# Martinsos/edlib

Measured on NVIDIA H100. Metric: GCUPS, higher is better.
Workload: dtype u32

## Files before the change

edlib_b200/csrc/eb_common.h:

```cpp
#pragma once
#include <stdint.h>

#if defined(__CUDACC__)
#define EB_HD __host__ __device__ __forceinline__
#define EB_D __device__ __forceinline__
#else
#define EB_HD inline
#define EB_D inline
#endif

namespace eb {

struct U2 { uint32_t x, y; };

constexpr int KPOS = 4;

struct Rec {
    int best;
    int cnt;
    int last;
    int rsv;
    int pos[KPOS];
};

// ... 211 lines not shown
    int maxLen;
    int Ls;
    int Lidx, sigma, numKeys;
    const int* bucketStart;
    const int* positions;
    int maxBucket;
    int level;
    int spread;
    int* winPair;
    int* winK;
    int* winStart;
    int* winLen;
    int* winTf;
    int winCap;
    int* winCount;
    SeedPlan* plan;
};
struct Leftover {
    int pair;
    int excl;
};
enum RecState : int { REC_DONE = 100, REC_PENDING = 101 };
struct WinReduceParams {
    const SeedPlan* plan;
    const WinRec* winRecs;
    int numReads;
    Rec* out;
    int* extra;
    int* extraCount;
    int extraCap;
    const Ovf* ovf;
    const int* ovfCount;
    int ovfCap;
    Leftover* leftover;
    int* leftoverCount;
    const int* readList;
    int firstPair;
    const int* qlen;
    int kBound;
};
struct FinParams {
    const Rec* recs;
    const int* extra;
    const int* readList;
    int firstPair;
    int numReads;
    const int* qlen;
    int kBound;
    int* ed;
    int* endCount;
    long long* endStart;
    int* cnt32;
    int* pool;
    long long poolBase;
    int poolCap;
    int* header;
    const int* winCount;
};

enum ResStage : int {
    RS_LOC_COUNT = 0,
    RS_LOC_JOBS = 1,
    RS_LOC_APPLY = 2,
    RS_PATH_FLAG = 3,
    RS_PATH_JOBS = 4,
    RS_PATH_LEN = 5,
// ... 68 lines not shown
```

edlib_b200/csrc/eb_core.h:

```cpp
#pragma once
#include "eb_common.h"

#if defined(__CUDA_ARCH__)
#define EB_UNROLL _Pragma("unroll")
#else
#define EB_UNROLL
#endif

namespace eb {


EB_HD uint32_t funnel_l1(uint32_t lo, uint32_t hi) {
#if defined(__CUDA_ARCH__)
    return __funnelshift_l(lo, hi, 1);
#else
    return (hi << 1) | (lo >> 31);
#endif
}

EB_HD int popcount32(uint32_t v) {
#if defined(__CUDA_ARCH__)
    return __popc(v);
#else
    return __builtin_popcount(v);
// ... 633 lines not shown
        if (bandSlack >= 0) {
            while (i < c && E[i] - first <= bandSlack) last = E[i++];
        } else {
            while (i < c && E[i] - last <= K1_RANGE_GAP && E[i] - first <= p.spread) last = E[i++];
        }
        int lo = first - t, hi = last + t;
        if (lo <= prevHi) lo = prevHi + 1;
        if (lo < 0) lo = 0;
        if (hi > p.n - 1) hi = p.n - 1;
        if (lo > hi) continue;
        prevHi = hi;
        int ws = lo - (m + t);
        if (ws < 0) ws = 0;
        ws &= ~15;
        f(nW, ws, lo, hi);
        ++nW;
    }
    return nW;
}
EB_HD void seed_window_store(const SeedPlanParams& p, int w, int pair, int t, int ws, int lo, int hi) {
    p.winPair[w] = pair;
    p.winK[w] = t + 1;
    p.winStart[w] = ws;
    p.winLen[w] = hi - ws + 1;
    p.winTf[w] = lo - ws;
}

struct CoopSerial {
    static constexpr int W = 1;
    static EB_HD int lane() { return 0; }
    static EB_HD int width() { return 1; }
    static EB_HD void sync() {}
    static EB_HD bool any(bool v) { return v; }
    static EB_HD int add_shared(int* p, int v) {
        const int old = *p;
        *p = old + v;
        return old;
    }
    static EB_HD int scan(int v, int& total) {
        total = v;
        return 0;
    }
    static EB_HD int reserve(int* counter, int n) { return n > 0 ? atomic_add_int(counter, n) : 0; }
};

EB_HD constexpr int seed_ctl_words(int W) { return 2 + 3 * W; }
constexpr int SEED_CTL = seed_ctl_words(32);

template <int CAP, int K, class C>
EB_HD void seed_try(const SeedPlanParams& p, const uint8_t* q, int m, int Lk, const int (&pos)[K], const int (&a)[K],
                    int* E, int* ctl) {
    bool same[K];
    EB_UNROLL
    for (int k = 0; k < K; ++k) {
        same[k] = pos[k] >= 0 && pos[k] + p.Ls <= p.n;
        if (same[k]) {
            uint32_t diff = 0;
            for (int x = Lk; x < p.Ls; ++x) diff |= (uint32_t)(p.tcodes[pos[k] + x] ^ q[a[k] + x]);
            same[k] = diff == 0;
        }
    }
    EB_UNROLL
    for (int k = 0; k < K; ++k) {
        if (!same[k]) continue;
        const int at = C::add_shared(&ctl[0], 1);
        if (at < CAP) E[at] = pos[k] + (m - a[k]) - 1;
// ... 99 lines not shown
                        }
                    }
                    C::sync();
                }
            }
        }
    }
    int myWs = 0, myLo = 0, myHi = 0;
    const int nW = seed_windows(p, E, c, m, t, [&](int w, int ws, int lo, int hi) {
        if (w == lane) {
            myWs = ws;
            myLo = lo;
            myHi = hi;
        }
    });
    const int base = C::reserve(p.winCount, nW);
    if (nW > 0) {
        if (base + nW <= p.winCap) {
            if (lane < nW) seed_window_store(p, base + lane, pair, t, myWs, myLo, myHi);
            if (nW > W)
                seed_windows(p, E, c, m, t, [&](int w, int ws, int lo, int hi) {
                    if (w >= W && w % W == lane) seed_window_store(p, base + w, pair, t, ws, lo, hi);
                });
            pl.first = base;
            pl.count = nW;
            pl.state = SEED_WINDOWS;
        } else {
            pl.state = SEED_SATURATED;
        }
    }
    if (live && lane == 0) p.plan[slot] = pl;
}

EB_HD void win_reduce_read(const WinReduceParams& p, int slot) {
    const SeedPlan pl = p.plan[slot];
    Rec out;
    out.best = 0x7fffffff;
    out.cnt = 0;
    out.last = 0;
    out.rsv = pl.state;
    for (int q = 0; q < KPOS; ++q) out.pos[q] = 0;
    if (pl.state == SEED_WINDOWS) {
        const int t = pl.thr;
        int b = 0x7fffffff;
        for (int w = 0; w < pl.count; ++w) {
            const WinRec& r = p.winRecs[pl.first + w];
            if (r.cnt > 0 && r.best < b) b = r.best;
        }
        if (b > t) {
            out.rsv = SEED_NONE;
        } else {
            int total = 0;
            bool longList = false, listed = false;
            for (int w = 0; w < pl.count; ++w) {
                const WinRec& r = p.winRecs[pl.first + w];
                if (r.cnt <= 0 || r.best != b) continue;
                if (r.cnt > KPOSW) listed = true;
                total += r.cnt;
            }
            int listLen = 0;
            if (listed) {
                listLen = p.ovfCap > 0 ? *p.ovfCount : 0x7fffffff;
                if (listLen > p.ovfCap) longList = true;
            }
            int base = 0;
            if (!longList && total > KPOS) {
                base = atomic_add_int(p.extraCount, total - KPOS);
                if (base + total - KPOS > p.extraCap) longList = true;
            }
            if (longList) {
                out.rsv = SEED_LONG_LIST;
            } else {
                int i = 0;
                for (int w = 0; w < pl.count; ++w) {
                    const WinRec& r = p.winRecs[pl.first + w];
                    if (r.cnt <= 0 || r.best != b) continue;
                    for (int q = 0; q < r.cnt && q < KPOSW; ++q, ++i) {
                        if (i < KPOS) out.pos[i] = r.pos[q];
                        else p.extra[base + i - KPOS] = r.pos[q];
                    }
                    if (r.cnt > KPOSW) {
                        int found = 0;
                        for (int e = 0; e < listLen; ++e) {
                            const Ovf o = p.ovf[e];
                            if (o.rec != pl.first + w || o.score != b) continue;
                            if (found < r.cnt - KPOSW) p.extra[base + i++ - KPOS] = o.pos;
                            ++found;
                        }
                        if (found != r.cnt - KPOSW) longList = true;
                    }
                }
                if (longList) {
                    out.rsv = SEED_LONG_LIST;
                } else {
                    out.best = b;
                    out.cnt = total;
                    out.last = base;
                }
            }
        }
    }
    if (p.leftover) {
        const int pair = p.readList ? p.readList[slot] : p.firstPair + slot;
        const int m = p.qlen[pair];
        const int bound = (p.kBound < 0 || p.kBound > m) ? m : p.kBound;
        int excl = -3;
        if (out.rsv == SEED_WINDOWS) {
            out.rsv = REC_DONE;
        } else if (out.rsv == SEED_NONE && pl.thr >= 0 && pl.thr == bound) {
            out.rsv = REC_DONE;
        } else {
            excl = out.rsv == SEED_LONG_LIST ? -2 : (out.rsv == SEED_NONE ? pl.thr : -1);
            out.rsv = REC_PENDING;
        }
        if (excl != -3) {
            const int at = atomic_add_int(p.leftoverCount, 1);
            p.leftover[at].pair = pair;
            p.leftover[at].excl = excl;
        }
    }
    p.out[slot] = out;
}

EB_HD int hw_accepted_count(int best, int cnt, int m, int kBound, bool* minusOne) {
    *minusOne = false;
    if (best < 0 || best == 0x7fffffff || cnt <= 0) return -1;
    if (kBound >= 0 && best > kBound) return -1;
    if (best > m) return -1;
    const int W64 = (m + 63) / 64 * 64 - m;
    *minusOne = (best == m && W64 > 0);
    return cnt + (*minusOne ? 1 : 0);
}
EB_HD void fin_count_item(const FinParams& p, int slot) {
    const Rec r = p.recs[slot];
// ... 744 lines not shown
```

edlib_b200/csrc/eb_engine.cpp:

```cpp
#include "eb_engine_internal.h"

#include <sched.h>

namespace eb {

static int env_int(const char* name, int dflt) {
    const char* s = getenv(name);
    return (s && *s) ? atoi(s) : dflt;
}

static std::vector<int> parse_cpulist(const char* path) {
    std::vector<int> cpus;
    FILE* f = fopen(path, "r");
    if (!f) return cpus;
    char buf[4096];
    if (fgets(buf, sizeof(buf), f)) {
        for (char* tok = strtok(buf, ",\n"); tok; tok = strtok(nullptr, ",\n")) {
            int a = 0, b = 0;
            const int got = sscanf(tok, "%d-%d", &a, &b);
            if (got == 1) b = a;
            if (got >= 1)
                for (int c = a; c <= b && c < 4096; ++c) cpus.push_back(c);
        }
    }
// ... 29 lines not shown
    snprintf(path, sizeof(path), "/sys/devices/system/node/node%d/cpulist", node);
    std::vector<int> cpus = parse_cpulist(path);
    if (!cpus.empty() && HostPool::worker_cpus().empty()) HostPool::worker_cpus() = cpus;
}

EngineTunables::EngineTunables() {
    k1MinGroup = env_int("EDLIB_B200_K1_MIN_GROUP", k1MinGroup);
    k1MinChunk = env_int("EDLIB_B200_K1_MIN_CHUNK", k1MinChunk);
    ovfCap = env_int("EDLIB_B200_OVF_CAP", ovfCap);
    filterK0 = env_int("EDLIB_B200_FILTER_K0", filterK0);
    filterK1 = env_int("EDLIB_B200_FILTER_K1", filterK1);
    packParallelBytes = (size_t)env_int("EDLIB_B200_PACK_PARALLEL_KB", (int)(packParallelBytes >> 10)) << 10;
    filterSeedK = env_int("EDLIB_B200_FILTER_SEED_K", filterSeedK);
    filterSeedBucket = env_int("EDLIB_B200_FILTER_SEED_BUCKET", filterSeedBucket);
    filterSeedSlack = env_int("EDLIB_B200_FILTER_SEED_SLACK", filterSeedSlack);
    filterMinLevelReads = env_int("EDLIB_B200_FILTER_MIN_LEVEL_READS", filterMinLevelReads);
    tinySweepReads = env_int("EDLIB_B200_TINY_SWEEP_READS", tinySweepReads);
    filterSeedLevels = std::min(SEED_LEVELS, env_int("EDLIB_B200_FILTER_SEED_LEVELS", filterSeedLevels));
    filterMaxWindows = env_int("EDLIB_B200_FILTER_MAX_WINDOWS", filterMaxWindows);
    filterMinLen = env_int("EDLIB_B200_FILTER_MIN_LEN", filterMinLen);
    filterSpread = env_int("EDLIB_B200_FILTER_SPREAD", filterSpread);
    filterMinTarget = env_int("EDLIB_B200_FILTER_MIN_TARGET", filterMinTarget);
    filterSkipRepeats = env_int("EDLIB_B200_FILTER_SKIP_REPEATS", filterSkipRepeats);
    bandKernel = env_int("EDLIB_B200_BAND_KERNEL", bandKernel);
    collapseEqualities = env_int("EDLIB_B200_COLLAPSE_EQUALITIES", collapseEqualities);
    directUpload = env_int("EDLIB_B200_DIRECT_UPLOAD", directUpload);
    streamSlices = std::max(1, env_int("EDLIB_B200_STREAM_SLICES", streamSlices));
    directMinBytes = (size_t)env_int("EDLIB_B200_DIRECT_MIN_KB", (int)(directMinBytes >> 10)) << 10;
    deviceStage = env_int("EDLIB_B200_DEVICE_STAGE", deviceStage);
    windowCheckAfter = env_int("EDLIB_B200_WINDOW_CHECK", windowCheckAfter);
    longHwMinTarget = env_int("EDLIB_B200_LONG_HW_MIN_TARGET", longHwMinTarget);
    longSeedMaxK = env_int("EDLIB_B200_LONG_SEED_MAX_K", longSeedMaxK);
    devSliceReads = std::max(64, env_int("EDLIB_B200_SLICE_READS", devSliceReads));
    streamMinPairs = env_int("EDLIB_B200_STREAM_MIN_PAIRS", streamMinPairs);
    const int sliceMb = env_int("EDLIB_B200_SLICE_MB", 0);
    if (sliceMb > 0) sliceBytes = (size_t)sliceMb << 20;
    if (sliceMb > 0) pathSliceBytes = (size_t)sliceMb << 20;
    deviceResults = env_int("EDLIB_B200_DEVICE_RESULTS", deviceResults);
}

static int code_map(const uint32_t (&present)[8], uint8_t (&map)[256], int other) {
    int ncodes = 0;
    for (int b = 0; b < 256; ++b) ncodes += (present[b >> 5] >> (b & 31)) & 1u;
    int next = 0;
    for (int b = 0; b < 256; ++b) {
        if (present[b >> 5] >> (b & 31) & 1u) map[b] = (uint8_t)next++;
        else map[b] = (uint8_t)(other < 0 ? 0 : std::min(other, 255));
    }
    return ncodes;
}

Prepared* Engine::prepare(const BatchInput& in) {
    Backend* be = be_;
    Trace trace;
    Prepared* p = spare_ ? spare_ : new Prepared();
    spare_ = nullptr;
    try {
        p->bind(be);
        p->tg.clear();
        p->hasEq = false;
        p->ncodes = 0;
        p->computed = false;
        p->classified = false;
        p->ed.clear();
        p->endStart.clear();
        p->endCount.clear();
// ... 1110 lines not shown
```

edlib_b200/csrc/eb_engine.h:

```cpp
#pragma once
#include <stddef.h>
#include <stdint.h>

#include <map>
#include <string>
#include <utility>
#include <vector>

#include "../../include/edlib.h"
#include "eb_common.h"

namespace eb {

struct Backend {
    virtual ~Backend() {}
    virtual void* alloc(size_t bytes) = 0;
    virtual void free(void* p) = 0;
    virtual void* alloc_host(size_t bytes) = 0;
    virtual void free_host(void* p) = 0;
    virtual bool host_pinned(const void* , size_t ) { return false; }
    virtual void h2d(void* dst, const void* src, size_t bytes) = 0;
    virtual void d2h(void* dst, const void* src, size_t bytes) = 0;
    virtual void zero(void* dst, size_t bytes) = 0;
    virtual void d2d(void* dst, const void* src, size_t bytes) = 0;
// ... 28 lines not shown
    virtual void launch_seed_count(const SeedIndexParams& p) = 0;
    virtual void launch_scan(int* data, int count) = 0;
    virtual void launch_seed_fill(const SeedIndexParams& p) = 0;
    virtual void launch_seed_plan(const SeedPlanParams& p) = 0;
    virtual void launch_win_reduce(const WinReduceParams& p) = 0;
    virtual void launch_fin_count(const FinParams& p) = 0;
    virtual void launch_fin_fill(const FinParams& p) = 0;
    virtual void launch_qalpha(const QAlphaParams& p) = 0;
    virtual void reset_timing() = 0;
    virtual double kernel_ms(const char* nameOrNull) = 0;
    virtual int launches() = 0;
    virtual std::string kernel_report() = 0;
};

struct BatchInput {
    const char* const* queries;
    const int* queryLengths;
    const char* const* targets;
    const int* targetLengths;
    int numPairs;
    EdlibAlignConfig config;
};

struct EngineTunables {
    int k1MinGroup = 32;
    int k1MinChunk = 1024;
    int ovfCap = 1 << 20;
    size_t sliceBytes = 1ull << 30;
    size_t pathSliceBytes = 8ull << 30;
    int deviceResults = 1;
    size_t packParallelBytes = 32u << 20;
    int deviceStage = 1;
    int devSliceReads = 1 << 20;
    int streamSlices = 8;
    int streamMinPairs = 32768;
    int longHwMinTarget = 65536;
    int longSeedMaxK = 1024;
    int windowCheckAfter = 48;
    int filterSeedK = 20;
    int filterSeedBucket = 128;
    int filterSeedLevels = 4;
    int tinySweepReads = 8;
    int filterMinLevelReads = 64;
    int filterSeedSlack = 4;
    int filterK1 = 8;
    int filterK0 = 16;
    int filterMinLen = 96;
    int filterSpread = 1024;
    int filterMaxWindows = 32;
    int filterMinTarget = 65536;
    size_t directMinBytes = 1u << 20;
    int directUpload = 1;
    int collapseEqualities = 1;
    int bandKernel = 1;
    int filterSkipRepeats = 1;
    EngineTunables();
};

struct EngineStats {
    double kernelMs = 0;
    double k1Ms = 0;
    int launches = 0;
    long long h2dBytes = 0, d2hBytes = 0;
    long long k1Cells = 0;
    long long wCells = 0;
    long long filterDecided = 0, filterFallback = 0;
// ... 47 lines not shown
```

edlib_b200/csrc/eb_engine_internal.h:

```cpp
#pragma once
#include "eb_engine.h"

#include <stdio.h>
#include <stdlib.h>
#include <string.h>

#include <algorithm>
#include <cmath>
#include <exception>
#include <functional>
#include <atomic>
#include <condition_variable>
#include <mutex>
#include <chrono>
#include <map>
#include <stdexcept>
#include <thread>
#include <unordered_map>

namespace eb {


struct Trace {
    bool on;
// ... 382 lines not shown
    int firstPair = -1;
    size_t listOff = 0;
    int count = 0;
    long long poolBase = 0;
    int poolCap = 0;
    int poolFetched = 0;
    uint64_t done = 0;
    bool finished = false;
};

struct Pass {
    Engine& eng;
    Backend* be;
    Prepared* p;
    EngineTunables& tun;
    EngineStats& stats;
    Trace trace;
    const int N, mode, k;
    std::vector<int>&best, &cnt;
    std::vector<long long>& posStart;
    std::vector<int>&posLen, &posPool;
    std::vector<int> wPairs;
    std::vector<uint8_t> opsPool;
    WRunner runner;
    int laneOkCache[9] = {-1, -1, -1, -1, -1, -1, -1, -1, -1};

    bool devMode = false;
    std::vector<int> hostPairs;
    std::vector<DevSlice> slices;
    DevBuf<int> dEd, dEndCount, dHeaders, dPool, dLeftCount, dLists;
    DevBuf<long long> dEndStart;
    DevBuf<Leftover> dLeft;
    PinnedVec<int> hHeaders;
    long long poolReserved = 0;
    size_t listsUsed = 0;
    bool wholeArrays = false;
    long long windowsSeen = 0, readsSeen = 0;
    void* extraCopyDst = nullptr;
    const void* extraCopySrc = nullptr;
    size_t extraCopyBytes = 0;

    Pass(Engine& e, Backend* b, Prepared* pr)
        : eng(e), be(b), p(pr), tun(e.tun), stats(e.stats), N(pr->N), mode(pr->mode), k(pr->cfg.k),
          best(e.scratch.best), cnt(e.scratch.cnt), posStart(e.scratch.posStart), posLen(e.scratch.posLen),
          posPool(e.scratch.posPool), runner{&e, b, pr, &opsPool} {
        hHeaders.bind(b);
        best.resize((size_t)N);
        cnt.resize((size_t)N);
        posStart.resize((size_t)N);
        posLen.resize((size_t)N);
        posPool.clear();
    }
    void host_touch(const int* list, size_t n) {
        parallel_ranges(n, 65536, [&](size_t lo, size_t hi) {
            for (size_t i = lo; i < hi; ++i) {
                const int pair = list[i];
                best[pair] = -1;
                cnt[pair] = 0;
                posStart[pair] = -1;
                posLen[pair] = 0;
            }
        });
    }
    void host_touch_all() {
        parallel_ranges((size_t)N, 65536, [&](size_t lo, size_t hi) {
            for (size_t i = lo; i < hi; ++i) {
                best[i] = -1;
                cnt[i] = 0;
                posStart[i] = -1;
                posLen[i] = 0;
            }
        });
    }

    bool lane_ok(int m);

    void lane_launch(const std::vector<LJob>& jobs, int nw, int laneMode, bool rev, std::vector<Rec>& recs);

    template <class Sink>
// ... 126 lines not shown
```

edlib_b200/csrc/eb_kernels.cu:

```cuda
#include <cuda_runtime.h>
#include <ctype.h>
#include <stdio.h>
#include <sys/syscall.h>
#include <unistd.h>
#include <stdlib.h>
#include <string.h>

#include <algorithm>
#include <mutex>
#include <stdexcept>
#include <string>
#include <vector>

#include "eb_core.h"
#include "eb_engine.h"

namespace eb {

#if defined(__CUDA_ARCH__)
#define EB_DEV(expr, fallback) expr
#else
#define EB_DEV(expr, fallback) fallback
#endif
struct DevWarp {
// ... 322 lines not shown
}

__global__ void traceback_kernel(const TbParams p) {
    const int job = blockIdx.x * blockDim.x + threadIdx.x;
    if (job < p.numJobs) traceback_job(p, job);
}

__global__ void res_kernel(const ResParams p) {
    const int i = blockIdx.x * blockDim.x + threadIdx.x;
    if (i < p.numItems) res_item(p, i);
}

__global__ void split_kernel(const SplitParams p) {
    const int node = blockIdx.x * blockDim.x + threadIdx.x;
    if (node < p.numNodes) split_node(p, node);
}

__global__ void seed_count_kernel(const SeedIndexParams p) {
    const int i = blockIdx.x * blockDim.x + threadIdx.x;
    if (i < p.numPos) seed_count_item(p, i);
}
__global__ void seed_fill_kernel(const SeedIndexParams p) {
    const int i = blockIdx.x * blockDim.x + threadIdx.x;
    if (i < p.numPos) seed_fill_item(p, i);
}
template <int GW>
struct CoopGroup {
    static constexpr int W = GW;
    static EB_D int lane() { return (int)(threadIdx.x & (GW - 1)); }
    static EB_D int width() { return GW; }
    static EB_D unsigned mask() { return GW == 32 ? 0xffffffffu : ((1u << (GW & 31)) - 1u) << (threadIdx.x & 31u & ~(GW - 1u)); }
    static EB_D void sync() { __syncwarp(mask()); }
    static EB_D bool any(bool v) { return __ballot_sync(mask(), v) != 0u; }
    static EB_D int add_shared(int* p, int v) { return atomicAdd(p, v); }
    static EB_D int scan(int v, int& total) {
        int incl = v;
        EB_UNROLL
        for (int d = 1; d < GW; d *= 2) {
            const int y = __shfl_up_sync(mask(), incl, d, GW);
            if (lane() >= d) incl += y;
        }
        total = __shfl_sync(mask(), incl, GW - 1, GW);
        return incl - v;
    }
    static EB_D int reserve(int* counter, int n) {
        const int l32 = (int)(threadIdx.x & 31u);
        int incl = n;
        EB_UNROLL
        for (int d = GW; d < 32; d *= 2) {
            const int y = __shfl_up_sync(0xffffffffu, incl, d);
            if (l32 >= d) incl += y;
        }
        const int total = __shfl_sync(0xffffffffu, incl, 31);
        int base = 0;
        if (total > 0) {
            if (l32 == 31) base = atomicAdd(counter, total);
            base = __shfl_sync(0xffffffffu, base, 31);
        }
        return base + incl - n;
    }
};
template <int CAP, int THREADS, class Group>
__global__ void __launch_bounds__(THREADS, 1536 / THREADS) seed_plan_kernel(const SeedPlanParams p) {
    extern __shared__ __align__(16) unsigned char smemRaw[];
    constexpr int GW = Group::W;
    constexpr int GROUPS = THREADS / GW;
    int* E = reinterpret_cast<int*>(smemRaw);
    int* ctl = E + GROUPS * CAP;
    const int g = threadIdx.x / GW;
    seed_plan_read<CAP, Group>(p, blockIdx.x * GROUPS + g, E + g * CAP, ctl + g * seed_ctl_words(GW));
}
__global__ void win_reduce_kernel(const WinReduceParams p) {
    const int slot = blockIdx.x * blockDim.x + threadIdx.x;
    if (slot < p.numReads) win_reduce_read(p, slot);
}
__global__ void fin_count_kernel(const FinParams p) {
    const int slot = blockIdx.x * blockDim.x + threadIdx.x;
    if (slot < p.numReads) fin_count_item(p, slot);
}
__global__ void fin_fill_kernel(const FinParams p) {
    const int slot = blockIdx.x * blockDim.x + threadIdx.x;
    if (slot < p.numReads) fin_fill_item(p, slot);
}
__global__ void qalpha_kernel(const QAlphaParams p) {
    const int q = blockIdx.x * (blockDim.x >> 5) + (threadIdx.x >> 5);
    if (q >= p.numQueries) return;
    uint32_t local[8];
    qalpha_scan(p, q, threadIdx.x & 31, 32, local);
    int total = 0;
#pragma unroll
    for (int k = 0; k < 8; ++k) total += __popc(__reduce_or_sync(0xffffffffu, local[k]) | p.tmask[k]);
    if ((threadIdx.x & 31) == 0) p.alphaLen[p.firstPair + q] = total;
}

constexpr int SCAN_THREADS = 256, SCAN_PER = 16, SCAN_TILE = SCAN_THREADS * SCAN_PER;
template <int THREADS>
__device__ int block_exclusive_scan(int v, int* total) {
    __shared__ int warpSums[32];
    const int lane = threadIdx.x & 31, wid = threadIdx.x >> 5;
    int incl = v;
#pragma unroll
    for (int d = 1; d < 32; d <<= 1) {
        const int o = __shfl_up_sync(0xffffffffu, incl, d);
        if (lane >= d) incl += o;
    }
    if (lane == 31) warpSums[wid] = incl;
    __syncthreads();
// ... 603 lines not shown
            EB_CUDA(cudaFuncSetAttribute(seed_plan_kernel<CAP, THREADS, CoopGroup<GW>>, cudaFuncAttributeMaxDynamicSharedMemorySize, (int)smem));
        seed_plan_kernel<CAP, THREADS, CoopGroup<GW>><<<(p.numReads + GROUPS - 1) / GROUPS, THREADS, smem, stream>>>(p);
    }
    void launch_seed_plan(const SeedPlanParams& p) override {
        Scope s(this, "seed_plan");
        const bool narrow = p.maxLen > 0 && p.Ls > 0 && std::min(p.maxLen / p.Ls, p.seedK + 1) <= 16;
        if (p.level <= 0) {
            if (narrow) launch_seed_plan_t<SEED_CAND_0, 128, 16>(p);
            else launch_seed_plan_t<SEED_CAND_0, 128, 32>(p);
        } else if (p.level == 1) {
            if (narrow) launch_seed_plan_t<SEED_CAND_1, 128, 16>(p);
            else launch_seed_plan_t<SEED_CAND_1, 128, 32>(p);
        } else {
            launch_seed_plan_t<SEED_CAND_2, 64, 32>(p);
        }
        check_launch("seed_plan");
    }
    void launch_fin_count(const FinParams& p) override {
        Scope s(this, "fin_count");
        fin_count_kernel<<<(p.numReads + 255) / 256, 256, 0, stream>>>(p);
        check_launch("fin_count");
    }
    void launch_fin_fill(const FinParams& p) override {
        Scope s(this, "fin_fill");
        fin_fill_kernel<<<(p.numReads + 255) / 256, 256, 0, stream>>>(p);
        check_launch("fin_fill");
    }
    void launch_qalpha(const QAlphaParams& p) override {
        Scope s(this, "qalpha");
        qalpha_kernel<<<(p.numQueries + 7) / 8, 256, 0, stream>>>(p);
        check_launch("qalpha");
    }
    void launch_win_reduce(const WinReduceParams& p) override {
        Scope s(this, "win_reduce");
        win_reduce_kernel<<<(p.numReads + 127) / 128, 128, 0, stream>>>(p);
        check_launch("win_reduce");
    }
    void launch_split(const SplitParams& p) override {
        Scope s(this, "split");
        split_kernel<<<(p.numNodes + 63) / 64, 64, 0, stream>>>(p);
        check_launch("split");
    }
    void launch_traceback(const TbParams& p) override {
        Scope s(this, "traceback");
        traceback_kernel<<<(p.numJobs + 127) / 128, 128, 0, stream>>>(p);
        check_launch("traceback");
    }
    void reset_timing() override {
        for (auto& t : timed) {
            pool.push_back(t.a);
            pool.push_back(t.b);
        }
        timed.clear();
        launchCount = 0;
    }
    double kernel_ms(const char* name) override {
        cudaStreamSynchronize(stream);
        double total = 0;
        for (auto& t : timed) {
            if (name && strcmp(name, t.name) != 0) continue;
            float ms = 0;
            if (cudaEventElapsedTime(&ms, t.a, t.b) == cudaSuccess) total += ms;
        }
        return total;
    }
    int launches() override { return launchCount; }
// ... 60 lines not shown
```

edlib_b200/csrc/eb_pass_lane.cpp:

```cpp
#include "eb_engine_internal.h"

namespace eb {

bool Pass::lane_ok(int m) {
    if (m <= 0 || m > 256) return false;
    const int nw = ceil_div(m, 32);
    if (laneOkCache[nw] < 0) {
        int bt = 0, rc = 0;
        be->k1_shape(nw, p->ncodes, 0x7fffffff, &bt, &rc);
        laneOkCache[nw] = rc > 0 ? 1 : 0;
    }
    return laneOkCache[nw] == 1;
}

void Pass::lane_launch(const std::vector<LJob>& jobs, int nw, int laneMode, bool rev, std::vector<Rec>& recs) {
    const size_t J = jobs.size();
    recs.resize(J);
    const size_t step = 4u << 20;
    for (size_t a = 0; a < J; a += step) {
        const size_t n = std::min(step, J - a);
        DevBuf<LJob> dJobs(be, n);
        dJobs.upload(jobs.data() + a, n);
        DevBuf<Rec> dRecs(be, n);
        be->zero(dRecs.p, n * sizeof(Rec));
// ... 315 lines not shown
        wp.kInit = wK.p;
        wp.winStart = wStart.p;
        wp.winLen = wLen.p;
        wp.trackFrom = wTf.p;
        wp.numReads = V;
        wp.checkAfter = tun.windowCheckAfter;
        wp.ncodes = p->ncodes;
        wp.eqtab = nullptr;
        wp.recs = dWinRecs.p;
        wp.ovf = dOvf.p;
        wp.ovfCount = dOvfCount.p;
        wp.ovfCap = ovfCap;
        be->launch_k1w(wp, nw);
    }
    DevBuf<Rec> dOut(be, g);
    int extraCap = g / 4 + 16384;
    DevBuf<int> dExtra;
    int nExtra = 0;
    for (;;) {
        dExtra.alloc(be, (size_t)extraCap);
        be->zero(dCount.p, sizeof(int));
        WinReduceParams rp;
        memset(&rp, 0, sizeof(rp));
        rp.plan = dPlan.p;
        rp.winRecs = dWinRecs.p;
        rp.numReads = g;
        rp.out = dOut.p;
        rp.extra = dExtra.p;
        rp.extraCount = dCount.p;
        rp.extraCap = extraCap;
        rp.ovf = dOvf.p;
        rp.ovfCount = dOvfCount.p;
        rp.ovfCap = ovfCap;
        be->launch_win_reduce(rp);
        dCount.download(&nExtra, 1);
        if (nExtra <= extraCap) break;
        extraCap = nExtra;
    }
    HostBuf<Rec> out(be, g);
    dOut.download(out.p, g);
    std::vector<int> extra((size_t)nExtra);
    if (nExtra) dExtra.download(extra.data(), (size_t)nExtra);
    stats.d2hBytes += (long long)g * (long long)sizeof(Rec) + 4 + 4LL * nExtra;
    trace.mark("filter: seed windows");
    struct Part {
        std::vector<int> next, direct;
        long long decided = 0, positions = 0;
        int nSat = 0, nLong = 0;
    };
    std::vector<Part> parts;
    std::vector<size_t> partLo;
    {
        const size_t nparts = host_parts((size_t)g, 65536);
        parts.resize(nparts);
        for (size_t t2 = 0; t2 <= nparts; ++t2) partLo.push_back((size_t)g * t2 / nparts);
    }
    auto for_parts = [&](const std::function<void(size_t)>& fn) { HostPool::get().run(parts.size(), fn); };
    for_parts([&](size_t t2) {
        Part& P = parts[t2];
        for (size_t i = partLo[t2]; i < partLo[t2 + 1]; ++i) {
            const int s = cand[i], pair = list[s];
            const Rec& r = out[i];
            if (thr[i] < 0) {
                P.next.push_back(s);
            } else if (r.rsv == SEED_WINDOWS) {
                P.decided++;
// ... 322 lines not shown
            if (stageP[st] / 32 >= nw) continue;
            std::vector<int> next;
            prefix_stage(c, stageP[st], stageK[st], cur, next);
            cur.swap(next);
        }
    }
    if (trace.on)
        fprintf(stderr, "[edlib_b200] plain sweep: %zu reads sent directly (long end-location lists, repeats), %zu undecided\n", c.direct.size(), cur.size());
    c.direct.insert(c.direct.end(), cur.begin(), cur.end());
    if (filtered) stats.filterFallback += (long long)c.direct.size();
    trace.mark("filter: collect");
    plain_sweep(c);
}

bool Pass::dev_eligible(int t, int nw) {
    (void)nw;
    if (mode != MODE_HW || p->hasEq || !tun.deviceStage) return false;
    if (tun.filterSeedK <= 0 || tun.filterSeedLevels <= 0) return false;
    if (p->tg[t].len < tun.filterMinTarget) return false;
    return true;
}

void Pass::dev_begin(int maxSlices) {
    devMode = true;
    dEd.alloc(be, (size_t)N);
    dEndCount.alloc(be, (size_t)N);
    dEndStart.alloc(be, (size_t)N);
    dLeft.alloc(be, (size_t)N);
    dLeftCount.alloc(be, 1);
    be->zero(dLeftCount.p, sizeof(int));
    dHeaders.alloc(be, (size_t)4 * maxSlices);
    be->zero(dHeaders.p, (size_t)4 * maxSlices * sizeof(int));
    hHeaders.resize((size_t)4 * maxSlices);
    slices.clear();
    slices.reserve((size_t)maxSlices);
    poolReserved = 0;
}

int Pass::dev_enqueue_slice(int t, int nw, int firstPair, const int* listHost, int first, int count) {
    const Target& tg = p->tg[t];
    if (!seed_index(t) || seedIdx->Ls[0] <= 0) throw std::runtime_error("internal: device stage without a seed index");
    const SeedIndex& sx = *seedIdx;
    const int si = (int)slices.size();
    DevSlice sl;
    sl.t = t;
    sl.nw = nw;
    sl.firstPair = firstPair >= 0 ? firstPair + first : -1;
    sl.count = count;
    sl.poolBase = poolReserved;
    sl.poolCap = 4 * count + count / 4 + DEV_EXTRA_SLACK;
    poolReserved += sl.poolCap;
    if (poolReserved > (long long)dPool.n) throw std::runtime_error("internal: end-location pool of the device stage too small");
    const int* dList = nullptr;
    if (firstPair < 0) {
        if (listsUsed + (size_t)count > dLists.n) throw std::runtime_error("internal: read lists of the device stage too small");
        be->h2d(dLists.p + listsUsed, listHost + first, (size_t)count * sizeof(int));
        dList = dLists.p + listsUsed;
        listsUsed += (size_t)count;
    }
    int& perRead = eng.scratch.seedWindowsPerRead[0];
    const int cap = (int)std::min<long long>((long long)count * std::max(perRead + 2, 6) + 4096, 1LL << 28);
    const int extraCap = count / 4 + DEV_EXTRA_SLACK;
    const int ovfCap = cap / 8 + 65536;
    DevBuf<Ovf> dOvf(be, (size_t)ovfCap);
    DevBuf<SeedPlan> dPlan(be, count);
    DevBuf<int> wPair(be, cap), wK(be, cap), wStart(be, cap), wLen(be, cap), wTf(be, cap);
// ... 50 lines not shown
    rp.ovf = dOvf.p;
    rp.ovfCount = dCtr.p + 2;
    rp.ovfCap = ovfCap;
    rp.leftover = dLeft.p;
    rp.leftoverCount = dLeftCount.p;
    rp.readList = dList;
    rp.firstPair = sl.firstPair;
    rp.qlen = p->dQlen.p;
    rp.kBound = k;
    be->launch_win_reduce(rp);
    FinParams fp;
    memset(&fp, 0, sizeof(fp));
    fp.recs = dOut.p;
    fp.extra = dExtra.p;
    fp.readList = dList;
    fp.firstPair = sl.firstPair;
    fp.numReads = count;
    fp.qlen = p->dQlen.p;
    fp.kBound = k;
    fp.ed = dEd.p;
    fp.endCount = dEndCount.p;
    fp.endStart = dEndStart.p;
    fp.cnt32 = dCnt32.p;
    fp.pool = dPool.p + sl.poolBase;
    fp.poolBase = sl.poolBase;
    fp.poolCap = sl.poolCap;
    fp.header = dHeaders.p + 4 * si;
    fp.winCount = dCtr.p;
    be->launch_fin_count(fp);
    be->launch_scan(dCnt32.p, count);
    be->launch_fin_fill(fp);
    const uint64_t done = be->mark(Backend::STREAM_COMPUTE);
    be->wait(Backend::STREAM_RESULTS, done);
    be->d2h_async(Backend::STREAM_RESULTS, hHeaders.data() + 4 * si, dHeaders.p + 4 * si, 4 * sizeof(int));
    sl.poolFetched = std::min(sl.poolCap, count + count / 4 + 1024);
    be->d2h_async(Backend::STREAM_RESULTS, p->endPool.data() + sl.poolBase, dPool.p + sl.poolBase, (size_t)sl.poolFetched * sizeof(int));
    if (sl.firstPair >= 0) {
        be->d2h_async(Backend::STREAM_RESULTS, p->ed.data() + sl.firstPair, dEd.p + sl.firstPair, (size_t)count * sizeof(int));
        be->d2h_async(Backend::STREAM_RESULTS, p->endCount.data() + sl.firstPair, dEndCount.p + sl.firstPair, (size_t)count * sizeof(int));
        be->d2h_async(Backend::STREAM_RESULTS, p->endStart.data() + sl.firstPair, dEndStart.p + sl.firstPair, (size_t)count * sizeof(long long));
        stats.d2hBytes += 16LL * count;
    } else {
        wholeArrays = true;
    }
    if (extraCopyBytes) {
        be->d2h_async(Backend::STREAM_RESULTS, extraCopyDst, extraCopySrc, extraCopyBytes);
        stats.d2hBytes += (long long)extraCopyBytes;
    }
    stats.d2hBytes += 16 + 4LL * sl.poolFetched;
    sl.done = be->mark(Backend::STREAM_RESULTS);
    slices.push_back(sl);
    return si;
}

void Pass::dev_finish_slice(int si) {
    DevSlice& sl = slices[(size_t)si];
    if (sl.finished) return;
    sl.finished = true;
    be->host_wait(sl.done);
    const int* h = hHeaders.data() + 4 * si;
    if (h[2]) throw std::runtime_error("internal: end-location pool region of a slice overflowed");
    if (h[0] > sl.poolFetched) {
        be->d2h(p->endPool.data() + sl.poolBase + sl.poolFetched, dPool.p + sl.poolBase + sl.poolFetched,
                (size_t)(h[0] - sl.poolFetched) * sizeof(int));
        stats.d2hBytes += 4LL * (h[0] - sl.poolFetched);
    }
    stats.filterWindows += h[3];
    stats.filterDecided += sl.count - h[1];
    windowsSeen += h[3];
    readsSeen += sl.count;
}

void Pass::dev_leftovers() {
    for (size_t si = 0; si < slices.size(); ++si) dev_finish_slice((int)si);
    if (readsSeen > 0) eng.scratch.seedWindowsPerRead[0] = (int)((windowsSeen + readsSeen - 1) / readsSeen);
    int L = 0;
    dLeftCount.download(&L, 1);
    if (wholeArrays) {
        be->d2h_async(Backend::STREAM_COMPUTE, p->ed.data(), dEd.p, (size_t)N * sizeof(int));
        be->d2h_async(Backend::STREAM_COMPUTE, p->endCount.data(), dEndCount.p, (size_t)N * sizeof(int));
        be->d2h_async(Backend::STREAM_COMPUTE, p->endStart.data(), dEndStart.p, (size_t)N * sizeof(long long));
        stats.d2hBytes += 16LL * N;
    }
    HostBuf<Leftover> left(be, (size_t)std::max(L, 1));
    if (L) be->d2h(left.p, dLeft.p, (size_t)L * sizeof(Leftover));
    else be->sync();
    stats.d2hBytes += 4 + 8LL * L;
    trace.mark("device stage: results on the host");
    if (L == 0) return;
    std::sort(left.p, left.p + L, [](const Leftover& a, const Leftover& b) { return a.pair < b.pair; });
    trace.mark("device stage: leftovers sorted");
    std::map<std::pair<int, int>, std::pair<std::vector<int>, std::vector<int>>> groups;
    for (int i = 0; i < L; ++i) {
        const int pair = left[i].pair;
        auto& g = groups[std::make_pair(p->tidx[pair], ceil_div(p->qlen[pair], 32))];
        g.first.push_back(pair);
        g.second.push_back(left[i].excl);
        hostPairs.push_back(pair);
    }
    trace.mark("device stage: leftovers grouped");
    for (auto& kv : groups) lane_group(kv.first.first, kv.first.second, kv.second.first, &kv.second.second, 1);
}
}
```

Before: 104.3 million.

## Parallelize window reduction across a warp and prefetch leftovers asynchronously

Window reduction at deeper seed levels now runs one warp per read. Lanes stride over windows, combine with warp min, scan and broadcast, and scan the overflow list cooperatively instead of serially. Separately, the leftover count and a head of the leftover list are copied asynchronously on the results stream after each slice. The host can then start grouping and running leftover lane work before finishing the remaining slice copies, and the whole-array copies move to the results stream. This adds warp-shuffle overhead for reads with few windows and a more intricate ordering of host waits.

```diff
diff --git a/edlib_b200/csrc/eb_common.h b/edlib_b200/csrc/eb_common.h
--- a/edlib_b200/csrc/eb_common.h
+++ b/edlib_b200/csrc/eb_common.h
@@ -267,6 +267,7 @@
     const Ovf* ovf;
     const int* ovfCount;
     int ovfCap;
+    int warpPerRead;
     Leftover* leftover;
     int* leftoverCount;
     const int* readList;
diff --git a/edlib_b200/csrc/eb_core.h b/edlib_b200/csrc/eb_core.h
--- a/edlib_b200/csrc/eb_core.h
+++ b/edlib_b200/csrc/eb_core.h
@@ -689,6 +689,8 @@
     static EB_HD int width() { return 1; }
     static EB_HD void sync() {}
     static EB_HD bool any(bool v) { return v; }
+    static EB_HD int min(int v) { return v; }
+    static EB_HD int bcast(int v, int ) { return v; }
     static EB_HD int add_shared(int* p, int v) {
         const int old = *p;
         *p = old + v;
@@ -854,7 +856,10 @@
     if (live && lane == 0) p.plan[slot] = pl;
 }
 
+template <class C = CoopSerial>
 EB_HD void win_reduce_read(const WinReduceParams& p, int slot) {
+    const int lane = C::lane();
+    constexpr int W = C::W;
     const SeedPlan pl = p.plan[slot];
     Rec out;
     out.best = 0x7fffffff;
@@ -865,21 +870,24 @@
     if (pl.state == SEED_WINDOWS) {
         const int t = pl.thr;
         int b = 0x7fffffff;
-        for (int w = 0; w < pl.count; ++w) {
+        for (int w = lane; w < pl.count; w += W) {
             const WinRec& r = p.winRecs[pl.first + w];
             if (r.cnt > 0 && r.best < b) b = r.best;
         }
+        b = C::min(b);
         if (b > t) {
             out.rsv = SEED_NONE;
         } else {
-            int total = 0;
+            int mine = 0, total = 0;
             bool longList = false, listed = false;
-            for (int w = 0; w < pl.count; ++w) {
+            for (int w = lane; w < pl.count; w += W) {
                 const WinRec& r = p.winRecs[pl.first + w];
                 if (r.cnt <= 0 || r.best != b) continue;
                 if (r.cnt > KPOSW) listed = true;
-                total += r.cnt;
-            }
+                mine += r.cnt;
+            }
+            C::scan(mine, total);
+            listed = C::any(listed);
             int listLen = 0;
             if (listed) {
                 listLen = p.ovfCap > 0 ? *p.ovfCount : 0x7fffffff;
@@ -887,31 +895,50 @@
             }
             int base = 0;
             if (!longList && total > KPOS) {
-                base = atomic_add_int(p.extraCount, total - KPOS);
+                if (lane == 0) base = atomic_add_int(p.extraCount, total - KPOS);
+                base = C::bcast(base, 0);
                 if (base + total - KPOS > p.extraCap) longList = true;
             }
             if (longList) {
                 out.rsv = SEED_LONG_LIST;
             } else {
-                int i = 0;
-                for (int w = 0; w < pl.count; ++w) {
-                    const WinRec& r = p.winRecs[pl.first + w];
-                    if (r.cnt <= 0 || r.best != b) continue;
-                    for (int q = 0; q < r.cnt && q < KPOSW; ++q, ++i) {
-                        if (i < KPOS) out.pos[i] = r.pos[q];
-                        else p.extra[base + i - KPOS] = r.pos[q];
+                int at = 0;
+                for (int w0 = 0; w0 < pl.count; w0 += W) {
+                    const int w = w0 + lane;
+                    const WinRec* r = w < pl.count ? &p.winRecs[pl.first + w] : nullptr;
+                    const int n = (r && r->cnt > 0 && r->best == b) ? r->cnt : 0;
+                    int round = 0;
+                    const int i = at + C::scan(n, round);
+                    for (int q = 0; q < n && q < KPOSW; ++q) {
+                        if (i + q < KPOS) out.pos[i + q] = r->pos[q];
+                        else p.extra[base + i + q - KPOS] = r->pos[q];
                     }
-                    if (r.cnt > KPOSW) {
+                    bool pending = n > KPOSW;
+                    while (C::any(pending)) {
+                        const int src = C::min(pending ? lane : W);
+                        const int rec = C::bcast(pl.first + w, src), want = C::bcast(n - KPOSW, src);
+                        const int dst = C::bcast(i + KPOSW, src);
+                        if (lane == src) pending = false;
                         int found = 0;
-                        for (int e = 0; e < listLen; ++e) {
-                            const Ovf o = p.ovf[e];
-                            if (o.rec != pl.first + w || o.score != b) continue;
-                            if (found < r.cnt - KPOSW) p.extra[base + i++ - KPOS] = o.pos;
-                            ++found;
+                        for (int e0 = 0; e0 < listLen; e0 += W) {
+                            const int e = e0 + lane;
+                            bool hit = false;
+                            int col = 0;
+                            if (e < listLen) {
+                                const Ovf o = p.ovf[e];
+                                hit = o.rec == rec && o.score == b;
+                                col = o.pos;
+                            }
+                            int hits = 0;
+                            const int k = found + C::scan(hit ? 1 : 0, hits);
+                            if (hit && k < want) p.extra[base + dst + k - KPOS] = col;
+                            found += hits;
                         }
-                        if (found != r.cnt - KPOSW) longList = true;
+                        if (found != want) longList = true;
                     }
+                    at += round;
                 }
+                for (int q = 0; q < KPOS; ++q) C::scan(out.pos[q], out.pos[q]);
                 if (longList) {
                     out.rsv = SEED_LONG_LIST;
                 } else {
@@ -922,6 +949,7 @@
             }
         }
     }
+    if (lane != 0) return;
     if (p.leftover) {
         const int pair = p.readList ? p.readList[slot] : p.firstPair + slot;
         const int m = p.qlen[pair];
diff --git a/edlib_b200/csrc/eb_engine.cpp b/edlib_b200/csrc/eb_engine.cpp
--- a/edlib_b200/csrc/eb_engine.cpp
+++ b/edlib_b200/csrc/eb_engine.cpp
@@ -85,6 +85,7 @@
     longHwMinTarget = env_int("EDLIB_B200_LONG_HW_MIN_TARGET", longHwMinTarget);
     longSeedMaxK = env_int("EDLIB_B200_LONG_SEED_MAX_K", longSeedMaxK);
     devSliceReads = std::max(64, env_int("EDLIB_B200_SLICE_READS", devSliceReads));
+    devLeftHead = std::max(0, env_int("EDLIB_B200_LEFT_HEAD", devLeftHead));
     streamMinPairs = env_int("EDLIB_B200_STREAM_MIN_PAIRS", streamMinPairs);
     const int sliceMb = env_int("EDLIB_B200_SLICE_MB", 0);
     if (sliceMb > 0) sliceBytes = (size_t)sliceMb << 20;
diff --git a/edlib_b200/csrc/eb_engine.h b/edlib_b200/csrc/eb_engine.h
--- a/edlib_b200/csrc/eb_engine.h
+++ b/edlib_b200/csrc/eb_engine.h
@@ -84,6 +84,7 @@
     size_t packParallelBytes = 32u << 20;
     int deviceStage = 1;
     int devSliceReads = 1 << 20;
+    int devLeftHead = 65536;
     int streamSlices = 8;
     int streamMinPairs = 32768;
     int longHwMinTarget = 65536;
diff --git a/edlib_b200/csrc/eb_engine_internal.h b/edlib_b200/csrc/eb_engine_internal.h
--- a/edlib_b200/csrc/eb_engine_internal.h
+++ b/edlib_b200/csrc/eb_engine_internal.h
@@ -438,6 +438,10 @@
     DevBuf<long long> dEndStart;
     DevBuf<Leftover> dLeft;
     PinnedVec<int> hHeaders;
+    PinnedVec<int> hLeftCount;
+    PinnedVec<Leftover> hLeftHead;
+    int leftHead = 0;
+    uint64_t leftMark = 0;
     long long poolReserved = 0;
     size_t listsUsed = 0;
     bool wholeArrays = false;
@@ -451,6 +455,8 @@
           best(e.scratch.best), cnt(e.scratch.cnt), posStart(e.scratch.posStart), posLen(e.scratch.posLen),
           posPool(e.scratch.posPool), runner{&e, b, pr, &opsPool} {
         hHeaders.bind(b);
+        hLeftCount.bind(b);
+        hLeftHead.bind(b);
         best.resize((size_t)N);
         cnt.resize((size_t)N);
         posStart.resize((size_t)N);
diff --git a/edlib_b200/csrc/eb_kernels.cu b/edlib_b200/csrc/eb_kernels.cu
--- a/edlib_b200/csrc/eb_kernels.cu
+++ b/edlib_b200/csrc/eb_kernels.cu
@@ -378,6 +378,8 @@
     static EB_D unsigned mask() { return GW == 32 ? 0xffffffffu : ((1u << (GW & 31)) - 1u) << (threadIdx.x & 31u & ~(GW - 1u)); }
     static EB_D void sync() { __syncwarp(mask()); }
     static EB_D bool any(bool v) { return __ballot_sync(mask(), v) != 0u; }
+    static EB_D int min(int v) { return __reduce_min_sync(mask(), v); }
+    static EB_D int bcast(int v, int src) { return __shfl_sync(mask(), v, src, GW); }
     static EB_D int add_shared(int* p, int v) { return atomicAdd(p, v); }
     static EB_D int scan(int v, int& total) {
         int incl = v;
@@ -419,6 +421,10 @@
 __global__ void win_reduce_kernel(const WinReduceParams p) {
     const int slot = blockIdx.x * blockDim.x + threadIdx.x;
     if (slot < p.numReads) win_reduce_read(p, slot);
+}
+__global__ void win_reduce_warp_kernel(const WinReduceParams p) {
+    const int slot = (int)((blockIdx.x * blockDim.x + threadIdx.x) >> 5);
+    if (slot < p.numReads) win_reduce_read<CoopGroup<32>>(p, slot);
 }
 __global__ void fin_count_kernel(const FinParams p) {
     const int slot = blockIdx.x * blockDim.x + threadIdx.x;
@@ -1088,6 +1094,12 @@
         check_launch("qalpha");
     }
     void launch_win_reduce(const WinReduceParams& p) override {
+        if (p.warpPerRead) {
+            Scope s(this, "win_reduce_warp");
+            win_reduce_warp_kernel<<<(p.numReads + 3) / 4, 128, 0, stream>>>(p);
+            check_launch("win_reduce_warp");
+            return;
+        }
         Scope s(this, "win_reduce");
         win_reduce_kernel<<<(p.numReads + 127) / 128, 128, 0, stream>>>(p);
         check_launch("win_reduce");
diff --git a/edlib_b200/csrc/eb_pass_lane.cpp b/edlib_b200/csrc/eb_pass_lane.cpp
--- a/edlib_b200/csrc/eb_pass_lane.cpp
+++ b/edlib_b200/csrc/eb_pass_lane.cpp
@@ -371,6 +371,7 @@
         rp.ovf = dOvf.p;
         rp.ovfCount = dOvfCount.p;
         rp.ovfCap = ovfCap;
+        rp.warpPerRead = level > 0 ? 1 : 0;
         be->launch_win_reduce(rp);
         dCount.download(&nExtra, 1);
         if (nExtra <= extraCap) break;
@@ -759,6 +760,10 @@
     dHeaders.alloc(be, (size_t)4 * maxSlices);
     be->zero(dHeaders.p, (size_t)4 * maxSlices * sizeof(int));
     hHeaders.resize((size_t)4 * maxSlices);
+    leftHead = std::min(N, tun.devLeftHead);
+    hLeftCount.resize(1);
+    hLeftHead.resize((size_t)std::max(leftHead, 1));
+    leftMark = 0;
     slices.clear();
     slices.reserve((size_t)maxSlices);
     poolReserved = 0;
@@ -875,6 +880,10 @@
     be->launch_fin_fill(fp);
     const uint64_t done = be->mark(Backend::STREAM_COMPUTE);
     be->wait(Backend::STREAM_RESULTS, done);
+    be->d2h_async(Backend::STREAM_RESULTS, hLeftCount.data(), dLeftCount.p, sizeof(int));
+    be->d2h_async(Backend::STREAM_RESULTS, hLeftHead.data(), dLeft.p, (size_t)leftHead * sizeof(Leftover));
+    leftMark = be->mark(Backend::STREAM_RESULTS);
+    stats.d2hBytes += 4 + 8LL * leftHead;
     be->d2h_async(Backend::STREAM_RESULTS, hHeaders.data() + 4 * si, dHeaders.p + 4 * si, 4 * sizeof(int));
     sl.poolFetched = std::min(sl.poolCap, count + count / 4 + 1024);
     be->d2h_async(Backend::STREAM_RESULTS, p->endPool.data() + sl.poolBase, dPool.p + sl.poolBase, (size_t)sl.poolFetched * sizeof(int));
@@ -915,33 +924,43 @@
 }
 
 void Pass::dev_leftovers() {
+    uint64_t wholeDone = 0;
+    if (wholeArrays) {
+        be->wait(Backend::STREAM_RESULTS, be->mark(Backend::STREAM_COMPUTE));
+        be->d2h_async(Backend::STREAM_RESULTS, p->ed.data(), dEd.p, (size_t)N * sizeof(int));
+        be->d2h_async(Backend::STREAM_RESULTS, p->endCount.data(), dEndCount.p, (size_t)N * sizeof(int));
+        be->d2h_async(Backend::STREAM_RESULTS, p->endStart.data(), dEndStart.p, (size_t)N * sizeof(long long));
+        wholeDone = be->mark(Backend::STREAM_RESULTS);
+        stats.d2hBytes += 16LL * N;
+    }
+    int L = 0;
+    if (!slices.empty()) {
+        be->host_wait(leftMark);
+        L = hLeftCount[0];
+    }
+    HostBuf<Leftover> left(be, (size_t)std::max(L, 1));
+    if (L) memcpy(left.p, hLeftHead.data(), (size_t)std::min(L, leftHead) * sizeof(Leftover));
+    if (L > leftHead) {
+        be->d2h(left.p + leftHead, dLeft.p + leftHead, (size_t)(L - leftHead) * sizeof(Leftover));
+        stats.d2hBytes += 8LL * (L - leftHead);
+    }
+    trace.mark("device stage: leftovers on the host");
+    if (L > 0) {
+        std::sort(left.p, left.p + L, [](const Leftover& a, const Leftover& b) { return a.pair < b.pair; });
+        std::map<std::pair<int, int>, std::pair<std::vector<int>, std::vector<int>>> groups;
+        for (int i = 0; i < L; ++i) {
+            const int pair = left[i].pair;
+            auto& g = groups[std::make_pair(p->tidx[pair], ceil_div(p->qlen[pair], 32))];
+            g.first.push_back(pair);
+            g.second.push_back(left[i].excl);
+            hostPairs.push_back(pair);
+        }
+        trace.mark("device stage: leftovers grouped");
+        for (auto& kv : groups) lane_group(kv.first.first, kv.first.second, kv.second.first, &kv.second.second, 1);
+    }
     for (size_t si = 0; si < slices.size(); ++si) dev_finish_slice((int)si);
+    if (wholeDone) be->host_wait(wholeDone);
     if (readsSeen > 0) eng.scratch.seedWindowsPerRead[0] = (int)((windowsSeen + readsSeen - 1) / readsSeen);
-    int L = 0;
-    dLeftCount.download(&L, 1);
-    if (wholeArrays) {
-        be->d2h_async(Backend::STREAM_COMPUTE, p->ed.data(), dEd.p, (size_t)N * sizeof(int));
-        be->d2h_async(Backend::STREAM_COMPUTE, p->endCount.data(), dEndCount.p, (size_t)N * sizeof(int));
-        be->d2h_async(Backend::STREAM_COMPUTE, p->endStart.data(), dEndStart.p, (size_t)N * sizeof(long long));
-        stats.d2hBytes += 16LL * N;
-    }
-    HostBuf<Leftover> left(be, (size_t)std::max(L, 1));
-    if (L) be->d2h(left.p, dLeft.p, (size_t)L * sizeof(Leftover));
-    else be->sync();
-    stats.d2hBytes += 4 + 8LL * L;
     trace.mark("device stage: results on the host");
-    if (L == 0) return;
-    std::sort(left.p, left.p + L, [](const Leftover& a, const Leftover& b) { return a.pair < b.pair; });
-    trace.mark("device stage: leftovers sorted");
-    std::map<std::pair<int, int>, std::pair<std::vector<int>, std::vector<int>>> groups;
-    for (int i = 0; i < L; ++i) {
-        const int pair = left[i].pair;
-        auto& g = groups[std::make_pair(p->tidx[pair], ceil_div(p->qlen[pair], 32))];
-        g.first.push_back(pair);
-        g.second.push_back(left[i].excl);
-        hostPairs.push_back(pair);
-    }
-    trace.mark("device stage: leftovers grouped");
-    for (auto& kv : groups) lane_group(kv.first.first, kv.first.second, kv.second.first, &kv.second.second, 1);
-}
-}
+}
+}
```

Result: faster. 114.6 million (median of 6 runs) (+9.9%).
